# databio/IGD

Measured on AMD Instinct MI355X. Metric: query-intervals/sec (igd search -q, hits-only) on roadmap-scale synthetic .igd, higher is better.
Workload: dtype int32; 1 GPU; BASELINE config 2: roadmap-scale synthetic IGD, 1900 files x 26316 intervals (53143736 tile records, 188505 tiles of 16384 bp, hg38 contigs) replicated per GPU + 1000000 position-sorted queries per step (seed 7), hits-only, queries and DB resident in HBM; queries_per_gpu=1000000, parallelism=query-sharded x1, grouping=sorted, query_layout=contig numbers + starts + ends (12 B/query; igd_hip_search_dev), collective=none

## Files before the change

igd_amd/csrc/engine/host_open.hpp:

```cpp
static thread_local igd_hip_db *t_arenaOwner = nullptr;

template <typename T>
static int dalloc(T **p, size_t n, int64_t *acct)
{
    *p = nullptr;
    if (n == 0) n = 1;
    if (t_arenaOwner && t_arenaOwner->arena) {
        igd_hip_db *o = t_arenaOwner;
        const size_t at = (o->arenaUsed + 255) & ~(size_t)255, bytes = n * sizeof(T);
        if (at + bytes <= o->arenaSize) {
            *p = (T *)(o->arena + at);
            o->arenaUsed = at + bytes;
            if (acct) *acct += (int64_t)bytes;
            return IGD_HIP_OK;
        }
    }
    hipError_t e = hipMalloc((void **)p, n * sizeof(T));
    if (e != hipSuccess) {
        set_err("hipMalloc", e, __FILE__, __LINE__);
        return IGD_HIP_ERR_NOMEM;
    }
    if (acct) *acct += (int64_t)(n * sizeof(T));
    return IGD_HIP_OK;
}
// ... 54 lines not shown
    *got = want;
    return p;
}
extern "C" void igd_hip_free(void *p)
{
    if (!p) return;
    size_t *hdr = (size_t *)((char *)p - 64);
    void *drop = nullptr;
    {
        std::lock_guard<std::mutex> lk(g_pinLock);
        if (g_pinCache && g_pinCacheBytes >= hdr[0]) drop = hdr;
        else { drop = g_pinCache; g_pinCache = hdr; g_pinCacheBytes = hdr[0]; }
    }
    if (drop) (void)hipHostFree(drop);
}
extern "C" const char *igd_hip_scan_kernel_name(void) { return "igd_scan_sorted"; }

extern "C" const char *igd_hip_last_scan_kernel(igd_hip_db *db)
{
    if (db && db->inner) return igd_hip_last_scan_kernel(db->inner);
    if (!db || db->epoch == 0) return "";
    if (db->lastMode == 2) return "igd_scan_tiles";
    if (db->lastDirect) return "igd_scan_direct";
    int32_t uns = 0;
    if (hipSetDevice(db->device) != hipSuccess || hipDeviceSynchronize() != hipSuccess ||
        hipMemcpy(&uns, db->d_ctl + CTL_UNSORTED, 4, hipMemcpyDeviceToHost) != hipSuccess) return "";
    if (uns == db->epoch) return "igd_scan_tiles";
    return db->lastPacked ? "igd_scan_sorted" : "igd_scan_tiles";
}

static double wall_s(void)
{
    struct timespec t;
    clock_gettime(CLOCK_MONOTONIC, &t);
    return (double)t.tv_sec + 1e-9 * (double)t.tv_nsec;
}
#define OPEN_PHASE(name) do { if (tim) { double t_ = wall_s(); fprintf(stderr, "[igd timing]   open: %-22s %8.1f ms\n", name, 1e3 * (t_ - t0)); t0 = t_; } } while (0)

static int build_retiled(igd_hip_db *db, const igd_hip_desc *d, int realShift, const std::vector<Unit> &units, int device)
{
    const int64_t n = db->nRec;
    std::vector<int32_t> st((size_t)n), en((size_t)n), ix((size_t)n), va;
    HIPCHK(hipMemcpy(st.data(), db->d_start, (size_t)n * 4, hipMemcpyDeviceToHost));
    HIPCHK(hipMemcpy(en.data(), db->d_end, (size_t)n * 4, hipMemcpyDeviceToHost));
    HIPCHK(hipMemcpy(ix.data(), db->d_idx, (size_t)n * 4, hipMemcpyDeviceToHost));
    if (db->gType == 1) { va.resize((size_t)n); HIPCHK(hipMemcpy(va.data(), db->d_value, (size_t)n * 4, hipMemcpyDeviceToHost)); }
// ... 71 lines not shown
            snprintf(g_err, sizeof g_err, "igd_hip_open: this libigd_hip.so is a measurement build (IGD_EXP=0x%x) that gives WRONG counts; "
                     "set IGD_HIP_ALLOW_EXP_BUILD=1 to use it anyway", igd_hip_build_flags());
            return IGD_HIP_ERR_ARG;
        }
        fprintf(stderr, "igd_hip: WARNING: measurement build IGD_EXP=0x%x -- counts are WRONG on purpose\n", igd_hip_build_flags());
    }
    std::thread warm;
    try {
        warm = std::thread([device]() {
            int n = 0;
            if (hipGetDeviceCount(&n) == hipSuccess && device >= 0 && device < n && hipSetDevice(device) == hipSuccess) (void)hipFree(nullptr);
        });
    } catch (...) { }
    struct JoinWarm { std::thread &t; ~JoinWarm() { if (t.joinable()) t.join(); } } joinWarm{warm};
    igd_hip_db *db = new igd_hip_db();
    db->device = device;
    {
        const char *fr = getenv("IGD_HIP_RANK");
        db->forceRank = fr && *fr ? atoi(fr) : -1;
        const char *fb = getenv("IGD_HIP_BIG");
        db->bigImage = fb && *fb == '1';
        const char *fd = getenv("IGD_HIP_DIRECT");
        db->forceDirect = fd && *fd ? atoi(fd) : -1;
        db->splitNoStage = getenv("IGD_HIP_SPLIT_NOSTAGE") != nullptr;
        db->splitNoBits = getenv("IGD_HIP_SPLIT_NOBITS") != nullptr;
        db->splitNoRegion = getenv("IGD_HIP_SPLIT_NOREGION") != nullptr;
        db->timing = tim;
    }
    db->nbp = d->nbp; db->gType = d->gType; db->nCtg = d->nCtg; db->nFiles = d->nFiles;
    db->nRec = d->nRecords;

    int64_t nT = 0;
    for (int c = 0; c < d->nCtg; c++) nT += d->nTile[c];
    bool jfits = true;
    for (int c = 0; c < d->nCtg; c++) jfits = jfits && d->nTile[c] < (1 << 27);
    if (nT >= (1 << 27) || !jfits) {
        snprintf(g_err, sizeof g_err, "igd_hip_open: too many tiles (%lld; the engine's limit is 2^27-1)", (long long)nT);
        delete db;
        return IGD_HIP_ERR_ARG;
    }
    db->nT = (int32_t)nT;
    std::vector<int64_t> tileOff((size_t)nT + 1);
    std::vector<int32_t> tileCnt((size_t)nT + 1), tileBd((size_t)nT + 1), ctgBase((size_t)d->nCtg + 1),
        ctgNTile((size_t)d->nCtg + 1), tileUnit0((size_t)nT + 1);
    std::vector<Unit> units;
    int64_t off = 0;
// ... 360 lines not shown
```

igd_amd/csrc/engine/host_search.hpp:

```cpp

static int ensure_workspace(igd_hip_db *db, int64_t nq, int pairBytes)
{
    int rc;
    if (nq > db->wsQueries) {
        HIPCHK(hipDeviceSynchronize());
        if (db->d_fix) (void)hipFree(db->d_fix);
        if (db->d_qw) (void)hipFree(db->d_qw);
        if (db->d_later) (void)hipFree(db->d_later);
        if (db->d_laterHdr) (void)hipFree(db->d_laterHdr);
        db->d_fix = nullptr; db->d_qw = nullptr; db->d_later = nullptr; db->d_laterHdr = nullptr;
        db->wsQueries = 0;
        if ((rc = dalloc(&db->d_fix, (size_t)nq * 2, nullptr)) != IGD_HIP_OK) return rc;
        if ((rc = dalloc(&db->d_qw, (size_t)nq + 64, nullptr)) != IGD_HIP_OK) return rc;
        if ((rc = dalloc(&db->d_later, (size_t)nq + 4096 + 64, nullptr)) != IGD_HIP_OK) return rc;
        if ((rc = dalloc(&db->d_laterHdr, 2 * ((size_t)nq / 256 + 2), nullptr)) != IGD_HIP_OK) return rc;
        db->wsQueries = nq;
    }
    if (pairBytes == 0 || (nq <= db->wsBucket && pairBytes <= db->pairBytes)) return IGD_HIP_OK;
    HIPCHK(hipDeviceSynchronize());
    const int64_t cap = nq > db->wsBucket ? nq : db->wsBucket;
    const int pb = pairBytes > db->pairBytes ? pairBytes : db->pairBytes;
    {
        void *ws[] = { db->d_pairs, db->d_long, db->d_spTable, db->d_spT, db->d_spSub };
        for (void *q : ws) if (q) (void)hipFree(q);
// ... 204 lines not shown
    const int mode = (flags & IGD_HIP_FLAG_SORTED) ? 1 : (flags & IGD_HIP_FLAG_BUCKET) ? 2 : 0;
    const int krule = rule | ((db->v.vshift >= 0 && db->vnest) ? 0x100 : 0);
    const bool packed = db->packed && !(flags & IGD_HIP_FLAG_EXACT) && (!useV || db->packedV);
    if (db->epoch >= 0x3fffffff || db->covStale) {
        HIPCHK(hipMemsetAsync(db->d_spill, 0, ((size_t)db->nT + 2) * 4, st));
        HIPCHK(hipMemsetAsync(db->d_cov, 0, 4 * IGD_COV_LEN(db->nT) * 4, st));
        HIPCHK(hipMemsetAsync(db->d_ctl + CTL_COV, 0, 4 * 4, st));
        if (db->d_spSub && db->spShift >= 0)
            HIPCHK(hipMemsetAsync(db->d_spSub + (((size_t)db->spCoarse * SPF_S) << db->spShift) + db->spCoarse, 0, (size_t)db->spCoarse * 4, st));
        if (!db->covStale) db->epoch = 0;
        db->covStale = false;
    }
    db->epoch++;
    struct StaleGuard { igd_hip_db *d; bool done; ~StaleGuard() { if (!done) d->covStale = true; } } guard{db, false};
    int slot = -1;
    if (db->evOn && db->evUsed < db->evMax && (db->evSeen++ % (db->evEvery > 0 ? db->evEvery : 1)) == 0) slot = db->evUsed++;
    const bool pipeEv = slot >= 0 && slot < IGD_PIPE_EVENTS;
    if (pipeEv) HIPCHK(hipEventRecord(db->ev[4 * slot + 0], st));
    u64 *zh = (flags & IGD_HIP_FLAG_ZERO_FIRST) ? (u64 *)d_hits : nullptr;
    u64 *zt = (flags & IGD_HIP_FLAG_ZERO_FIRST) ? (u64 *)d_total : nullptr;
    const bool direct = mode == 1 && packed && db->ldsHits && db->nWin == 1 && db->v.tileD != nullptr && db->v.vshift < 0 && db->v.shift >= 0 && db->nCtg <= QB_CTG &&
                        (db->forceDirect > 0 || (db->forceDirect < 0 && (flags & IGD_HIP_FLAG_SHORT) && nq >= 28ll * db->nT));
    db->lastDirect = direct ? 1 : 0;
    if (mode != 2) {
        bool vec = ((((uintptr_t)d_ichr) | ((uintptr_t)d_qs) | ((uintptr_t)d_qe)) & 15) == 0;
        const bool fast = packed && db->v.shift >= 0 && db->nCtg <= QB_CTG;
        if (nq < 65536) vec = false;
        bool runsK = d_runs != nullptr && vec && fast;
        if (d_runs && !runsK) {
            if (nq > db->runCap) {
                HIPCHK(hipStreamSynchronize(st));
                if (db->d_runIchr) (void)hipFree(db->d_runIchr);
                db->d_runIchr = nullptr; db->runCap = 0;
                if ((rc = dalloc(&db->d_runIchr, (size_t)nq, nullptr)) != IGD_HIP_OK) return rc;
                db->runCap = nq;
            }
            k_expand_runs<<<(int)((nq + 255) / 256), 256, 0, st>>>(d_runs, db->nCtg, db->d_runIchr, (int)nq);
            d_ichr = db->d_runIchr;
            vec = vec && (((uintptr_t)d_ichr) & 15) == 0;
        }
        const int fillBlocks = (int)((db->nT >> 10) < 256 ? (db->nT >> 10) + 1 : 256);
        const bool wide = vec && nq >= ((int64_t)1 << 22);
#define QB_GRID(PER_) ((int)((nq + (PER_) - 1) / (PER_)) > fillBlocks ? (int)((nq + (PER_) - 1) / (PER_)) : fillBlocks)
#define QB_LAUNCH(VEC_, FAST_, WGT_)                                                                                                  \
    if (direct && FAST_ && runsK && VEC_ == 4)                                         \
        k_query_bounds<4, true, WGT_, true, true><<<QB_GRID(WGT_ * 4), WGT_, 0, st>>>(db->v, d_runs, d_qs, d_qe, (int)nq, krule,      \
        1, db->d_firstQ, db->d_lpos, db->d_fix, db->d_ctl, db->epoch, zh, zt, db->d_qw, db->d_later, db->d_spill,                      \
        (int2 *)db->d_laterHdr, 1);                                                                                                  \
    else if (direct && FAST_)                                                                                                        \
        k_query_bounds<VEC_, true, WGT_, false, true><<<QB_GRID(WGT_ * VEC_), WGT_, 0, st>>>(db->v, d_ichr, d_qs, d_qe, (int)nq, krule, \
        1, db->d_firstQ, db->d_lpos, db->d_fix, db->d_ctl, db->epoch, zh, zt, db->d_qw, db->d_later, db->d_spill,                      \
        (int2 *)db->d_laterHdr, 1);                                                                                                  \
    else if (runsK && VEC_ == 4 && FAST_)                                                                                             \
        k_query_bounds<4, true, WGT_, true><<<QB_GRID(WGT_ * 4), WGT_, 0, st>>>(db->v, d_runs, d_qs, d_qe, (int)nq, krule,            \
        packed ? 1 : 0, db->d_firstQ, db->d_lpos, db->d_fix, db->d_ctl, db->epoch, zh, zt, db->d_qw, db->d_later, db->d_spill,         \
        (int2 *)db->d_laterHdr, mode == 1 ? 1 : 0);                                                                                  \
    else                                                                                                                             \
    k_query_bounds<VEC_, FAST_, WGT_><<<QB_GRID(WGT_ * VEC_), WGT_, 0, st>>>(db->v, d_ichr, d_qs, d_qe, (int)nq, krule,               \
        packed ? 1 : 0, db->d_firstQ, db->d_lpos, db->d_fix, db->d_ctl, db->epoch, zh, zt, db->d_qw, db->d_later, db->d_spill,         \
        (int2 *)db->d_laterHdr, mode == 1 ? 1 : 0)
        if (wide && !direct) { if (fast) QB_LAUNCH(4, true, 1024); else QB_LAUNCH(4, false, 1024); }
        else if (vec) { if (fast) QB_LAUNCH(4, true, 256); else QB_LAUNCH(4, false, 256); }
        else { if (fast) QB_LAUNCH(1, true, 256); else QB_LAUNCH(1, false, 256); }
#undef QB_LAUNCH
#undef QB_GRID
        db->lbShift = wide ? 12 : vec ? 10 : 8;
    }
    if (mode != 1) {
        if (db->spShift >= 0)
            rc = launch_split(db, d_ichr, d_qs, d_qe, (int)nq, krule, mode == 2 ? 0 : db->epoch, packed ? 1 : 0, st,
                              mode == 2 ? zh : nullptr, mode == 2 ? zt : nullptr);
        else
            rc = launch_bucket(db, d_ichr, d_qs, d_qe, (int)nq, krule, mode == 2 ? 0 : db->epoch, packed ? 1 : 0, st,
                                      mode == 2 ? zh : nullptr, mode == 2 ? zt : nullptr);
        if (rc != IGD_HIP_OK) return rc;
    }
    const bool extEv = slot >= 0 && mode == 1 && packed && db->ldsHits && db->nWin == 1;
    if (slot >= 0 && !extEv) HIPCHK(hipEventRecord(db->ev[4 * slot + 1], st));
    ScanArgs a;
    a.firstQ = db->d_firstQ; a.pairN = db->d_pairN; a.pairPos = db->d_pairPos; a.pairs = (const int2 *)db->d_pairs;
    a.walkList = nullptr; a.ctl = db->d_ctl; a.q_ichr = d_ichr; a.q_qs = d_qs; a.q_qe = d_qe; a.q_w = db->d_qw;
    a.total = (u64 *)d_total; a.hitsOut = (u64 *)d_hits;
    a.nq = (int)nq; a.v = v; a.rule = rule; a.epoch = db->epoch; a.mode = mode;
    a.packedWalk = packed ? (useV ? 2 : 1) : 0;
    const int valves = direct ? 8 : (mode != 1 && packed && db->spShift >= 0 ? 1 : 0) | (mode != 2 && packed ? 2 : 0) |
                       (db->bigImage || db->nRec + IGD_CHUNK >= (1ll << 30) ? 4 : 0);
    const size_t tailWave = direct ? (size_t)IGD_D_WLDS : (size_t)IGD_WLDS_BYTES;
    size_t tailLds = (valves & (2 | 8)) ? (size_t)(db->ldsHits ? IGD_TAIL_WG / IGD_WAVE : 4) * tailWave : 0;
    int tailHistOff = -1;
    if ((size_t)db->nFiles * 8 <= (size_t)48 * 1024) { tailHistOff = (int)tailLds; tailLds += (size_t)db->nFiles * 8; }
    if (db->ldsHits) {
        a.out = db->d_slab;
        const SortK K = make_sortk(db, a);
        for (int win = 0; win < db->nWin; win++) {
            const bool last = win == db->nWin - 1;
            const int fileLo = win * db->winN, fileN = db->nWin == 1 ? db->nFiles : (db->nFiles - fileLo < db->winN ? db->nFiles - fileLo : db->winN);
            if (extEv) { db->evStart = db->ev[4 * slot + 1]; db->evStop = db->ev[4 * slot + 2]; }
            if (direct) {
                DirK D;
                D.db = db->v;
                D.a.firstQ = db->d_firstQ; D.a.tileD = db->v.tileD; D.a.q_qs = d_qs; D.a.q_qe = d_qe; D.a.ctl = db->d_ctl; D.a.fix = db->d_fix;
                D.a.heavyS = db->d_heavy + IGD_HEAVY_MAX; D.a.farList = db->d_far; D.a.nq = (int)nq; D.a.v = v; D.a.epoch = db->epoch;
                D.a.rule = rule; D.a.promised = 1; D.a.sbCap = db->sbCap; D.a.wldsBytes = IGD_D_WLDS + 2 * db->sbCap;
                D.a.out = db->d_slab; D.a.hitsOut = (u64 *)d_hits; D.a.totalOut = (u64 *)d_total;
                if (useV) launch_sorted(db, igd_scan_direct<true>, db->grid, IGD_WG_DIR, (size_t)db->ldsDirect, st, D);
                else launch_sorted(db, igd_scan_direct<false>, db->grid, IGD_WG_DIR, (size_t)db->ldsDirect, st, D);
            } else
            launch_scan_any<true>(db, a, useV, packed, st, db->nWin > 1 ? win : -1);
            if (extEv && db->evStart) {
                db->evStart = db->evStop = nullptr;
                HIPCHK(hipEventRecord(db->ev[4 * slot + 1], st)); HIPCHK(hipEventRecord(db->ev[4 * slot + 2], st));
            }
            if (slot >= 0 && last && !extEv) HIPCHK(hipEventRecord(db->ev[4 * slot + 2], st));
            ScanArgs w = a;
            w.out = (u64 *)d_hits;
            SortK Kt = K;
            Kt.a.sbCap = 0; Kt.a.wldsBytes = (int)tailWave; Kt.a.tailHistOff = tailHistOff;
            const int gx = (fileN + IGD_TAIL_WG - 1) / IGD_TAIL_WG;
            dim3 rg(gx, (!last || IGD_REDUCE_GROUPS * gx >= IGD_TAIL_WGS) ? IGD_REDUCE_GROUPS : (IGD_TAIL_WGS + gx - 1) / gx);
            const int rows32 = (mode != 2 && packed) ? db->epoch : 0;
            if (useV)
                k_reduce_slabs<true><<<rg, IGD_TAIL_WG, last ? tailLds : 0, st>>>(Kt, db->d_slab, db->grid, fileN, (u64 *)d_hits + fileLo, (u64 *)d_total,
                                                               db->d_ctl, mode == 1 ? db->epoch : 0, w, db->d_fix, db->d_long, db->d_heavy, last ? valves : -1, rows32);
            else
                k_reduce_slabs<false><<<rg, IGD_TAIL_WG, last ? tailLds : 0, st>>>(Kt, db->d_slab, db->grid, fileN, (u64 *)d_hits + fileLo, (u64 *)d_total,
                                                                db->d_ctl, mode == 1 ? db->epoch : 0, w, db->d_fix, db->d_long, db->d_heavy, last ? valves : -1, rows32);
        }
    } else {
        a.out = (u64 *)d_hits;
// ... 135 lines not shown
```

igd_amd/csrc/engine/measure.hpp:

```cpp
__global__ void k_unit_traffic(DbView db, const int32_t *__restrict__ firstQ, const int32_t *__restrict__ pairN,
                               const int32_t *__restrict__ spill, int epoch, int path ,
                               int rankOK, u64 *__restrict__ acc )
{
    const int u = blockIdx.x * blockDim.x + threadIdx.x;
    u64 nu = 0, nr = 0, np = 0, nd = 0;
    if (u < db.nUnits) {
        const Unit un = db.units[u];
        if (un.n > 0) {
            const int lj = UNIT_J(un);
            const int lb = lj < IGD_SHORT_TILES - 1 ? lj : IGD_SHORT_TILES - 1;
            const bool firstUnit = UNIT_FLAGS(un) & 1;
            if (path == 1) {
                if (firstQ[un.tile + 1] > firstQ[un.tile - lb]) { nu = 1; nr = (u64)un.n; }
            } else if (path == 2) {
                const int f0 = firstQ[un.tile], c0 = firstQ[un.tile + 1] - f0;
                const int cl = spill[un.tile] == epoch ? f0 - firstQ[un.tile - lb] : 0;
                if (c0 | cl) { nu = 1; nr = (u64)un.n; }
                if (firstUnit) {
                    if (rankOK && c0 >= IGD_DENSE_MIN) nd = (u64)c0;
                }
            } else if (pairN[un.tile] != 0) {
                nu = 1; nr = (u64)un.n;
                if (firstUnit) np = (u64)(pairN[un.tile] < 0 ? -pairN[un.tile] : pairN[un.tile]);
            }
// ... 9 lines not shown
        if (nd) atomicAdd(&acc[3], nd);
    }
}

__global__ void k_unit_traffic_direct(DbView db, const int32_t *__restrict__ firstQ, int rule, u64 *__restrict__ acc )
{
    const int u = blockIdx.x * blockDim.x + threadIdx.x;
    u64 nu = 0, nr = 0, nd = 0;
    if (u < db.nUnits) {
        const Unit un = db.units[u];
        const int c0 = firstQ[un.tile + 1] - firstQ[un.tile];
        const bool first = UNIT_FLAGS(un) & 1;
        if (c0 > 0 && c0 <= IGD_HEAVY_FIRST && (un.n > 0 || first)) {
            nd = (u64)c0;
            const bool dead = rule == IGD_HIP_RULE_NEST && un.n == 0;
            if (un.n > 0 || !dead) { nu = 1; nr = (u64)un.n + (first && !dead ? (u64)(db.tileD[un.tile].y & 127) : 0); }
        }
    }
    for (int o = 32; o > 0; o >>= 1) { nu += __shfl_down(nu, o); nr += __shfl_down(nr, o); nd += __shfl_down(nd, o); }
    if ((threadIdx.x & 63) == 0) {
        if (nu) atomicAdd(&acc[0], nu);
        if (nr) atomicAdd(&acc[1], nr);
        if (nd) atomicAdd(&acc[3], nd);
    }
}

extern "C" int igd_hip_batch_traffic(igd_hip_db *db, const int32_t *d_ichr, const int32_t *d_qs, const int32_t *d_qe,
                                     int64_t nq, int32_t v, int rule, int flags, igd_hip_traffic *out)
{
    if (!db || !out || nq < 0 || nq > IGD_MAX_BATCH) return IGD_HIP_ERR_ARG;
    if (db->inner) {
        db->inner->vnest = rule == IGD_HIP_RULE_NEST ? 1 : 0;
        return igd_hip_batch_traffic(db->inner, d_ichr, d_qs, d_qe, nq, v, IGD_HIP_RULE_FLAT, flags, out);
    }
    memset(out, 0, sizeof *out);
    if (nq == 0 || db->nT == 0 || db->nFiles == 0) return IGD_HIP_OK;
    HIPCHK(hipSetDevice(db->device));
    u64 *d_acc = nullptr;
    int64_t *d_h = nullptr;
    int rc;
    if (db->promised && (rc = igd_hip_sync(db, db->stream)) != IGD_HIP_OK) return rc;
    if ((rc = dalloc(&d_acc, 4, nullptr)) != IGD_HIP_OK) return rc;
    if ((rc = dalloc(&d_h, (size_t)db->nFiles + 1, nullptr)) != IGD_HIP_OK) { (void)hipFree(d_acc); return rc; }
    hipStream_t st = db->stream;
    (void)hipMemsetAsync(d_acc, 0, 32, st);
    (void)hipMemsetAsync(d_h, 0, ((size_t)db->nFiles + 1) * 8, st);
    const bool saved = db->evOn;
    db->evOn = false;
    rc = igd_hip_search_dev(db, d_ichr, d_qs, d_qe, nq, v, rule, flags & ~IGD_HIP_FLAG_ZERO_FIRST, d_h, nullptr, st);
    db->evOn = saved;
    int32_t ctl[4] = {0, 0, 0, 0};
    hipError_t e = hipStreamSynchronize(st);
    if (e == hipSuccess) e = hipMemcpy(ctl, db->d_ctl, sizeof ctl, hipMemcpyDeviceToHost);
    if (rc == IGD_HIP_OK && e == hipSuccess) {
        const int mode = (flags & IGD_HIP_FLAG_SORTED) ? 1 : (flags & IGD_HIP_FLAG_BUCKET) ? 2 : 0;
        const bool sortedPath = mode == 1 || (mode == 0 && ctl[CTL_UNSORTED] != db->epoch);
        const bool useV = (v != IGD_HIP_NO_VALUE_FILTER && db->gType == 1);
        const bool packed = db->packed && !(flags & IGD_HIP_FLAG_EXACT) && (!useV || db->packedV);
        const int path = !sortedPath ? 0 : packed ? 2 : 1;
        const bool direct = db->lastDirect != 0 && sortedPath;
        if (direct) k_unit_traffic_direct<<<(db->nUnits + 255) / 256, 256, 0, st>>>(db->v, db->d_firstQ, rule, d_acc);
        else
        k_unit_traffic<<<(db->nUnits + 255) / 256, 256, 0, st>>>(db->v, db->d_firstQ, db->d_pairN, db->d_spill, db->epoch, path,
                                                               ctl[CTL_NOTSTART] != db->epoch ? 1 : 0, d_acc);
        u64 acc[4] = {0, 0, 0, 0};
        e = hipStreamSynchronize(st);
        if (e == hipSuccess) e = hipMemcpy(acc, d_acc, 32, hipMemcpyDeviceToHost);
        const int recB = packed ? (useV ? 8 : 6) : (useV ? 16 : 12);
        out->units = (int64_t)acc[0];
        out->records = (int64_t)acc[1];
        out->record_bytes = (int64_t)acc[1] * recB;
        out->unit_bytes = (int64_t)sizeof(Unit) * db->nUnits + (path == 2 ? 8ll * (db->nT + 1) : sortedPath ? 4ll * (db->nT + 1) : 8ll * db->nT);
        if (direct) out->unit_bytes = (int64_t)(sizeof(Unit) + 8 + 16) * db->nUnits;
        int64_t nLaterWords = 0;
        if (path == 2 && !direct) {
            const int64_t nb = (nq + ((int64_t)1 << db->lbShift) - 1) >> db->lbShift;
            std::vector<int32_t> hdr((size_t)nb * 2);
            e = hipMemcpy(hdr.data(), db->d_laterHdr, (size_t)nb * 8, hipMemcpyDeviceToHost);
            for (int64_t b = 0; b < nb; b++) nLaterWords += hdr[(size_t)b * 2];
        }
        out->query_bytes = direct ? 8ll * (int64_t)acc[3] : path == 2 ? 4ll * nq + 4ll * nLaterWords + 4ll * (int64_t)acc[3]
                         : path == 1 ? 12ll * nq : 8ll * (int64_t)acc[2];
        out->slab_bytes = db->ldsHits ? (int64_t)db->grid * db->nFiles * (path == 2 ? 4 : 8) : 8ll * db->nFiles;
        out->total = out->record_bytes + out->unit_bytes + out->query_bytes + out->slab_bytes;
    }
    (void)hipFree(d_acc); (void)hipFree(d_h);
    (void)igd_hip_sync(db, st);
    if (rc != IGD_HIP_OK) return rc;
    if (e != hipSuccess) { set_err("batch_traffic", e, __FILE__, __LINE__); return IGD_HIP_ERR_DEVICE; }
    return IGD_HIP_OK;
}

__global__ __launch_bounds__(256) void k_copy16(const float4 *__restrict__ in, float4 *__restrict__ outp, size_t n)
{
    size_t i = (size_t)blockIdx.x * blockDim.x + threadIdx.x;
    const size_t stride = (size_t)gridDim.x * blockDim.x;
    for (; i + 3 * stride < n; i += 4 * stride) {
        const float4 a = in[i], b = in[i + stride], c = in[i + 2 * stride], d = in[i + 3 * stride];
        outp[i] = a; outp[i + stride] = b; outp[i + 2 * stride] = c; outp[i + 3 * stride] = d;
    }
    for (; i < n; i += stride) outp[i] = in[i];
}
__global__ __launch_bounds__(256) void k_read16(const float4 *__restrict__ in, size_t n, float *__restrict__ sink)
{
// ... 128 lines not shown
```

igd_amd/csrc/engine/tail.hpp:

```cpp
struct TailHist {
    igd_lds_u64 *p;
    bool on;
    __device__ __forceinline__ void add(int ix, u64 v) const { (void)__hip_atomic_fetch_add(p + ix, v, __ATOMIC_RELAXED, __HIP_MEMORY_SCOPE_WORKGROUP); }
};

template <bool USE_V>
__device__ __forceinline__ void exact_walk_body(const DbView &db, const ScanArgs &a, const int2 *__restrict__ fixList,
                                                const int2 *__restrict__ longList, int gwave, int nwaves, int ctlv, const TailHist hist)
{
    const bool uns = __builtin_amdgcn_readlane(ctlv, CTL_UNSORTED) == a.epoch;
    if (a.mode == 1 && uns) return;
    const bool sortedPath = a.mode == 1 || (a.mode == 0 && !uns);
    const int2 *list = sortedPath ? fixList : longList;
    const int nList = __builtin_amdgcn_readlane(ctlv, (sortedPath ? CTL_NFIX : CTL_NLONG) + (a.epoch & 1));
    const int lane = threadIdx.x & 63;
    u64 found = 0;
    int per = (nList + nwaves - 1) / nwaves;
    per = per > IGD_WAVE ? IGD_WAVE : per;
    for (int l0 = gwave * per; l0 < nList; l0 += nwaves * per) {
        const int cnt = nList - l0 < per ? nList - l0 : per;
        int vq = 0, vkind = -1, vqs = 0, vqe = 0, vn1 = 0, vj1 = -1, vbase = 0, vcnt = 0, voffLo = 0, voffHi = 0, vlob = 0;
        int vu0 = 0, vnu = 0, vqe2 = 0;
        UnitRegs vur;
        vur.offLo = vur.offHi = vur.tile = vur.n = vur.jf = 0;
// ... 329 lines not shown
        if (!(wa.mode == 1 && uns) && (nList > 0 || cov)) {
            hist.on = true;
            for (int f = threadIdx.x; f < K.db.nFiles; f += blockDim.x) hist.p[f] = 0;
            __syncthreads();
        }
    }
    if (!(IGD_EXP & 0x100000)) exact_walk_body<USE_V>(K.db, wa, fixList, longList, gwave, nwaves, ctlv, hist);
    if (!(IGD_EXP & 0x200000)) coverage_body<USE_V>(K.db, wa, d_hits, d_total, gwave, nwaves, ctlv, hist);
    if (hist.on) {
        __syncthreads();
        for (int f = threadIdx.x; f < K.db.nFiles; f += blockDim.x) {
            const u64 c = hist.p[f];
            if (c) atomicAdd(&d_hits[f], c);
        }
    }
    if (valves & 1) heavy_bucket_body<USE_V>(K.db, wa, heavyB, d_hits, d_total, gwave, nwaves, lane, ctlv);
    if (valves & 8) {
        DirArgs d;
        d.firstQ = K.a.firstQ; d.tileD = K.db.tileD; d.q_qs = wa.q_qs; d.q_qe = wa.q_qe; d.ctl = K.a.ctlw; d.fix = nullptr;
        d.heavyS = K.a.heavyS; d.farList = K.a.farList; d.nq = wa.nq; d.v = wa.v; d.epoch = wa.epoch; d.rule = wa.rule;
        d.promised = 1; d.sbCap = 0; d.wldsBytes = K.a.wldsBytes; d.out = nullptr; d.hitsOut = d_hits; d.totalOut = d_total;
        direct_tail_body<USE_V>(K.db, d, smem + (size_t)(threadIdx.x >> 6) * (size_t)K.a.wldsBytes, gwave, nwaves, lane, ctlv);
    } else
    if (valves & 2) {
        unsigned char *wsm = smem + (size_t)(threadIdx.x >> 6) * (size_t)K.a.wldsBytes;
        if (valves & 4) heavy_sorted_body<USE_V, true>(K, d_hits, d_total, wsm, gwave, nwaves, lane, ctlv);
        else {
            const int par = wa.epoch & 1;
            const bool work = (__builtin_amdgcn_readlane(ctlv, CTL_NHEAVYS + par) | __builtin_amdgcn_readlane(ctlv, CTL_NFAR + par)) != 0 &&
                              __builtin_amdgcn_readlane(ctlv, CTL_UNSORTED) != wa.epoch;
            igd_lds_u64 *lh = (K.a.tailHistOff >= 0 && work) ? hist.p : nullptr;
            if (lh) {
                __syncthreads();
                for (int f = threadIdx.x; f < K.db.nFiles; f += blockDim.x) lh[f] = 0;
                __syncthreads();
            }
            if (!(IGD_EXP & 0x10000)) heavy_sorted_body<USE_V, false>(K, d_hits, d_total, wsm, gwave, nwaves, lane, ctlv, lh);
            if (!(IGD_EXP & 0x20000)) far_units_body<USE_V, false>(K, d_hits, d_total, wsm, gwave, nwaves, lane, ctlv, lh);
            if (lh) {
                __syncthreads();
                for (int f = threadIdx.x; f < K.db.nFiles; f += blockDim.x) {
                    const u64 c = lh[f];
                    if (c) atomicAdd(&d_hits[f], c);
                }
            }
        }
// ... 76 lines not shown
```

igd_amd/csrc/igd_hip.hip:

```cpp
#include <hip/hip_runtime.h>
#include <hip/hip_ext.h>
#include <stdint.h>
#include <stdio.h>
#include <stdlib.h>
#include <string.h>
#include <limits.h>
#include <vector>
#include <algorithm>
#include <thread>
#include <mutex>
#include <time.h>
#include <unistd.h>

#include "igd_hip.h"
#include "igd_sortscan.hpp"

#define IGD_WAVE 64
#ifndef IGD_SLOTS
#define IGD_SLOTS 5
#endif
#define IGD_CHUNK (IGD_WAVE * IGD_SLOTS)
#define IGD_SHORT_TILES 4
#ifndef IGD_WPE
#define IGD_WPE 8
// ... 126 lines not shown
    int32_t *d_lpos;
    int32_t *d_cov;
    bool covStale;
    igd_hip_db *inner;
    uint32_t *d_rEmpty;
    int vnest;
    int32_t *d_runIchr;
    int64_t runCap;
    int32_t *d_qw;
    int32_t *d_later;
    int32_t *d_spill;
    int ldsSorted;
    int32_t maxTileCnt;
    int sbCap;
    int32_t *d_laterHdr;
    int lbShift;
    int lastMode, lastPacked;
    int forceRank;
    int forceDirect;
    int4 *d_tileD;
    uint32_t *d_tileBits;
    int ldsDirect;
    int lastDirect;
    bool bigImage;
    bool timing;
    bool splitNoStage, splitNoBits, splitNoRegion;
    uint32_t *d_spTable;
    SpTuple *d_spT;
    uint32_t *d_spSub;
    int spShift, spCoarse;
    char *arena;
    size_t arenaSize, arenaUsed;
    int32_t epoch;
    int32_t promised;
    int32_t *d_pairCnt, *d_pairPos, *d_blockSums;
    void *d_pairs;
    int2 *d_long, *d_fix;
    int32_t *d_ctl;
    int64_t wsQueries;
    int64_t wsBucket;
    int pairBytes;
    u64 *d_slab;
    int grid, ldsBytes;
    bool ldsHits;
    int winN, nWin;
    int64_t *d_qcount, *d_qoff, *d_enumBsum;
// ... 25 lines not shown
    unsigned *d_rsBits;
    int64_t rsUniCap, rsTabCap, rsSizeCap, rsBitsCap;
    u64 *d_coCols, *d_coMat, *d_coA, *d_coB;
    int64_t coColsCap, coMatCap, coACap, coBCap;
    int32_t *d_pmReg;
    long long *d_pmStat;
    int64_t pmRegCap, pmStatCap;
    hipStream_t stream;
    std::vector<hipEvent_t> ev;
    int evMax, evUsed;
    hipEvent_t evStart, evStop;
    int evEvery, evSeen;
    bool evOn;
};


#include "engine/upload.hpp"
#include "engine/query_bounds.hpp"
#include "engine/split.hpp"
#include "engine/compact_image.hpp"
#include "engine/scan_tiles.hpp"
#include "engine/scan_sorted.hpp"
#include "engine/scan_direct.hpp"
#include "engine/tail.hpp"
#include "engine/enumerate_dev.hpp"
#include "engine/hitmap_dev.hpp"
#include "engine/batch_stats_dev.hpp"
#include "engine/sets_dev.hpp"
#include "engine/support_dev.hpp"
#include "engine/coverage_dev.hpp"
#include "engine/member_dev.hpp"
#include "engine/fisher_dev.hpp"
#include "engine/rank_dev.hpp"
#include "engine/restrict_dev.hpp"
#include "engine/cooccur_dev.hpp"
#include "engine/permute_dev.hpp"
#include "engine/host_open.hpp"
#include "engine/host_search.hpp"
#include "engine/host_group.hpp"
#include "engine/host_enumerate.hpp"
#include "engine/seqpare.hpp"
#include "engine/host_misc.hpp"
#include "engine/host_sets.hpp"
#include "engine/host_support.hpp"
#include "engine/host_coverage.hpp"
#include "engine/host_member.hpp"
// ... 11 lines not shown
```

Baseline: 12.78 billion query-intervals/s.

## Add lean short-query scan kernel for sparse sorted query batches

Adds igd_scan_lean_short, a scan path for short, sparse, position-sorted queries. Each wave walks tile units and reads its query range straight from firstQ, instead of going through the later/spill pairing workspace. Heavy tiles and far-previous ranges are pushed to lists that a tail pass handles in slices. Query bounds run in the same bounds-only mode as the direct kernel, and the path is gated by query density thresholds plus an env override. The new path adds code complexity and atomics for the heavy and far lists, and it may only trigger for some batch sizes.

```diff
diff --git a/igd_amd/csrc/engine/host_open.hpp b/igd_amd/csrc/engine/host_open.hpp
--- a/igd_amd/csrc/engine/host_open.hpp
+++ b/igd_amd/csrc/engine/host_open.hpp
@@ -100,6 +100,7 @@
     if (!db || db->epoch == 0) return "";
     if (db->lastMode == 2) return "igd_scan_tiles";
     if (db->lastDirect) return "igd_scan_direct";
+    if (db->lastLeanShort) return "igd_scan_lean_short";
     int32_t uns = 0;
     if (hipSetDevice(db->device) != hipSuccess || hipDeviceSynchronize() != hipSuccess ||
         hipMemcpy(&uns, db->d_ctl + CTL_UNSORTED, 4, hipMemcpyDeviceToHost) != hipSuccess) return "";
@@ -217,6 +218,8 @@
         db->bigImage = fb && *fb == '1';
         const char *fd = getenv("IGD_HIP_DIRECT");
         db->forceDirect = fd && *fd ? atoi(fd) : -1;
+        const char *fl = getenv("IGD_HIP_LEAN_SHORT");
+        db->forceLeanShort = fl && *fl ? atoi(fl) : -1;
         db->splitNoStage = getenv("IGD_HIP_SPLIT_NOSTAGE") != nullptr;
         db->splitNoBits = getenv("IGD_HIP_SPLIT_NOBITS") != nullptr;
         db->splitNoRegion = getenv("IGD_HIP_SPLIT_NOREGION") != nullptr;
diff --git a/igd_amd/csrc/engine/host_search.hpp b/igd_amd/csrc/engine/host_search.hpp
--- a/igd_amd/csrc/engine/host_search.hpp
+++ b/igd_amd/csrc/engine/host_search.hpp
@@ -250,6 +250,16 @@
     const bool direct = mode == 1 && packed && db->ldsHits && db->nWin == 1 && db->v.tileD != nullptr && db->v.vshift < 0 && db->v.shift >= 0 && db->nCtg <= QB_CTG &&
                         (db->forceDirect > 0 || (db->forceDirect < 0 && (flags & IGD_HIP_FLAG_SHORT) && nq >= 28ll * db->nT));
     db->lastDirect = direct ? 1 : 0;
+    bool leanShort = false;
+    if (!direct && mode == 1 && (flags & IGD_HIP_FLAG_SHORT) && packed && db->ldsHits && db->nWin == 1 && db->v.tileD != nullptr && db->v.vshift < 0 &&
+        db->v.shift >= 0 && db->nCtg <= QB_CTG && db->nFiles > 8 && db->forceLeanShort != 0 && db->forceRank <= 0) {
+        const int64_t wavesLean = (int64_t)db->grid * (IGD_WG_LEAN / IGD_WAVE);
+        const bool fits = ((int64_t)db->nUnits + wavesLean - 1) / wavesLean * (IGD_WG_LEAN / IGD_WAVE) * (2 * IGD_LEAN_FIRST) * IGD_CHUNK < (1ll << 32);
+        const bool sparse = db->forceRank == 0 || (nq < 28ll * db->nT && nq >= (int64_t)db->nT);
+        leanShort = fits && (db->forceLeanShort > 0 || (sparse && nq >= (int64_t)(useV ? IGD_LEAN_SHORT_MIN_NQ_V : IGD_LEAN_SHORT_MIN_NQ)));
+    }
+    db->lastLeanShort = leanShort ? 1 : 0;
+    const bool bonly = direct || leanShort;
     if (mode != 2) {
         bool vec = ((((uintptr_t)d_ichr) | ((uintptr_t)d_qs) | ((uintptr_t)d_qe)) & 15) == 0;
         const bool fast = packed && db->v.shift >= 0 && db->nCtg <= QB_CTG;
@@ -271,11 +281,11 @@
         const bool wide = vec && nq >= ((int64_t)1 << 22);
 #define QB_GRID(PER_) ((int)((nq + (PER_) - 1) / (PER_)) > fillBlocks ? (int)((nq + (PER_) - 1) / (PER_)) : fillBlocks)
 #define QB_LAUNCH(VEC_, FAST_, WGT_)                                                                                                  \
-    if (direct && FAST_ && runsK && VEC_ == 4)                                         \
+    if (bonly && FAST_ && runsK && VEC_ == 4)                                         \
         k_query_bounds<4, true, WGT_, true, true><<<QB_GRID(WGT_ * 4), WGT_, 0, st>>>(db->v, d_runs, d_qs, d_qe, (int)nq, krule,      \
         1, db->d_firstQ, db->d_lpos, db->d_fix, db->d_ctl, db->epoch, zh, zt, db->d_qw, db->d_later, db->d_spill,                      \
         (int2 *)db->d_laterHdr, 1);                                                                                                  \
-    else if (direct && FAST_)                                                                                                        \
+    else if (bonly && FAST_)                                                                                                         \
         k_query_bounds<VEC_, true, WGT_, false, true><<<QB_GRID(WGT_ * VEC_), WGT_, 0, st>>>(db->v, d_ichr, d_qs, d_qe, (int)nq, krule, \
         1, db->d_firstQ, db->d_lpos, db->d_fix, db->d_ctl, db->epoch, zh, zt, db->d_qw, db->d_later, db->d_spill,                      \
         (int2 *)db->d_laterHdr, 1);                                                                                                  \
@@ -287,7 +297,7 @@
     k_query_bounds<VEC_, FAST_, WGT_><<<QB_GRID(WGT_ * VEC_), WGT_, 0, st>>>(db->v, d_ichr, d_qs, d_qe, (int)nq, krule,               \
         packed ? 1 : 0, db->d_firstQ, db->d_lpos, db->d_fix, db->d_ctl, db->epoch, zh, zt, db->d_qw, db->d_later, db->d_spill,         \
         (int2 *)db->d_laterHdr, mode == 1 ? 1 : 0)
-        if (wide && !direct) { if (fast) QB_LAUNCH(4, true, 1024); else QB_LAUNCH(4, false, 1024); }
+        if (wide && !bonly) { if (fast) QB_LAUNCH(4, true, 1024); else QB_LAUNCH(4, false, 1024); }
         else if (vec) { if (fast) QB_LAUNCH(4, true, 256); else QB_LAUNCH(4, false, 256); }
         else { if (fast) QB_LAUNCH(1, true, 256); else QB_LAUNCH(1, false, 256); }
 #undef QB_LAUNCH
@@ -311,7 +321,7 @@
     a.total = (u64 *)d_total; a.hitsOut = (u64 *)d_hits;
     a.nq = (int)nq; a.v = v; a.rule = rule; a.epoch = db->epoch; a.mode = mode;
     a.packedWalk = packed ? (useV ? 2 : 1) : 0;
-    const int valves = direct ? 8 : (mode != 1 && packed && db->spShift >= 0 ? 1 : 0) | (mode != 2 && packed ? 2 : 0) |
+    const int valves = direct ? 8 : leanShort ? 16 : (mode != 1 && packed && db->spShift >= 0 ? 1 : 0) | (mode != 2 && packed ? 2 : 0) |
                        (db->bigImage || db->nRec + IGD_CHUNK >= (1ll << 30) ? 4 : 0);
     const size_t tailWave = direct ? (size_t)IGD_D_WLDS : (size_t)IGD_WLDS_BYTES;
     size_t tailLds = (valves & (2 | 8)) ? (size_t)(db->ldsHits ? IGD_TAIL_WG / IGD_WAVE : 4) * tailWave : 0;
@@ -333,6 +343,16 @@
                 D.a.out = db->d_slab; D.a.hitsOut = (u64 *)d_hits; D.a.totalOut = (u64 *)d_total;
                 if (useV) launch_sorted(db, igd_scan_direct<true>, db->grid, IGD_WG_DIR, (size_t)db->ldsDirect, st, D);
                 else launch_sorted(db, igd_scan_direct<false>, db->grid, IGD_WG_DIR, (size_t)db->ldsDirect, st, D);
+            } else
+            if (leanShort) {
+                LsK S;
+                S.db = db->v;
+                S.a.firstQ = db->d_firstQ; S.a.q_qs = d_qs; S.a.q_qe = d_qe; S.a.ctl = db->d_ctl; S.a.fix = db->d_fix;
+                S.a.heavyS = db->d_heavy + IGD_HEAVY_MAX; S.a.farList = db->d_far; S.a.nq = (int)nq; S.a.v = v; S.a.epoch = db->epoch;
+                S.a.rule = rule; S.a.out = db->d_slab; S.a.hitsOut = (u64 *)d_hits; S.a.totalOut = (u64 *)d_total;
+                const size_t l = ((size_t)db->nFiles * 4 + 15) & ~(size_t)15;
+                if (useV) launch_sorted(db, igd_scan_lean_short<true>, db->grid, IGD_WG_LEAN, l, st, S);
+                else launch_sorted(db, igd_scan_lean_short<false>, db->grid, IGD_WG_LEAN, l, st, S);
             } else
             launch_scan_any<true>(db, a, useV, packed, st, db->nWin > 1 ? win : -1);
             if (extEv && db->evStart) {
diff --git a/igd_amd/csrc/engine/measure.hpp b/igd_amd/csrc/engine/measure.hpp
--- a/igd_amd/csrc/engine/measure.hpp
+++ b/igd_amd/csrc/engine/measure.hpp
@@ -55,6 +55,24 @@
         if (nu) atomicAdd(&acc[0], nu);
         if (nr) atomicAdd(&acc[1], nr);
         if (nd) atomicAdd(&acc[3], nd);
+    }
+}
+
+__global__ void k_unit_traffic_lean_short(DbView db, const int32_t *__restrict__ firstQ, int rule, u64 *__restrict__ acc )
+{
+    const int u = blockIdx.x * blockDim.x + threadIdx.x;
+    u64 nu = 0, nr = 0;
+    if (u < db.nUnits) {
+        const Unit un = db.units[u];
+        if (un.n > 0) {
+            const bool hasPrev = UNIT_J(un) > 0 && !(rule == IGD_HIP_RULE_NEST && (UNIT_FLAGS(un) & 2));
+            if (firstQ[un.tile + 1] > firstQ[un.tile - (hasPrev ? 1 : 0)]) { nu = 1; nr = (u64)un.n; }
+        }
+    }
+    for (int o = 32; o > 0; o >>= 1) { nu += __shfl_down(nu, o); nr += __shfl_down(nr, o); }
+    if ((threadIdx.x & 63) == 0) {
+        if (nu) atomicAdd(&acc[0], nu);
+        if (nr) atomicAdd(&acc[1], nr);
     }
 }
 
@@ -92,6 +110,9 @@
         const bool packed = db->packed && !(flags & IGD_HIP_FLAG_EXACT) && (!useV || db->packedV);
         const int path = !sortedPath ? 0 : packed ? 2 : 1;
         const bool direct = db->lastDirect != 0 && sortedPath;
+        const bool leanShort = db->lastLeanShort != 0 && sortedPath;
+        if (leanShort) k_unit_traffic_lean_short<<<(db->nUnits + 255) / 256, 256, 0, st>>>(db->v, db->d_firstQ, rule, d_acc);
+        else
         if (direct) k_unit_traffic_direct<<<(db->nUnits + 255) / 256, 256, 0, st>>>(db->v, db->d_firstQ, rule, d_acc);
         else
         k_unit_traffic<<<(db->nUnits + 255) / 256, 256, 0, st>>>(db->v, db->d_firstQ, db->d_pairN, db->d_spill, db->epoch, path,
@@ -106,13 +127,14 @@
         out->unit_bytes = (int64_t)sizeof(Unit) * db->nUnits + (path == 2 ? 8ll * (db->nT + 1) : sortedPath ? 4ll * (db->nT + 1) : 8ll * db->nT);
         if (direct) out->unit_bytes = (int64_t)(sizeof(Unit) + 8 + 16) * db->nUnits;
         int64_t nLaterWords = 0;
-        if (path == 2 && !direct) {
+        if (leanShort) out->unit_bytes = (int64_t)(sizeof(Unit) + 12) * db->nUnits;
+        if (path == 2 && !direct && !leanShort) {
             const int64_t nb = (nq + ((int64_t)1 << db->lbShift) - 1) >> db->lbShift;
             std::vector<int32_t> hdr((size_t)nb * 2);
             e = hipMemcpy(hdr.data(), db->d_laterHdr, (size_t)nb * 8, hipMemcpyDeviceToHost);
             for (int64_t b = 0; b < nb; b++) nLaterWords += hdr[(size_t)b * 2];
         }
-        out->query_bytes = direct ? 8ll * (int64_t)acc[3] : path == 2 ? 4ll * nq + 4ll * nLaterWords + 4ll * (int64_t)acc[3]
+        out->query_bytes = leanShort ? 8ll * nq : direct ? 8ll * (int64_t)acc[3] : path == 2 ? 4ll * nq + 4ll * nLaterWords + 4ll * (int64_t)acc[3]
                          : path == 1 ? 12ll * nq : 8ll * (int64_t)acc[2];
         out->slab_bytes = db->ldsHits ? (int64_t)db->grid * db->nFiles * (path == 2 ? 4 : 8) : 8ll * db->nFiles;
         out->total = out->record_bytes + out->unit_bytes + out->query_bytes + out->slab_bytes;
diff --git a/igd_amd/csrc/engine/scan_lean_short.hpp b/igd_amd/csrc/engine/scan_lean_short.hpp
--- /dev/null
+++ b/igd_amd/csrc/engine/scan_lean_short.hpp
@@ -0,0 +1,327 @@
+#ifndef IGD_LEAN_SHORT_MIN_NQ
+#define IGD_LEAN_SHORT_MIN_NQ 2000000
+#define IGD_LEAN_SHORT_MIN_NQ_V 1000000
+#endif
+#define WALK_WHOLE 5
+
+struct LsArgs {
+    const int32_t *firstQ;
+    const int32_t *q_qs, *q_qe;
+    int32_t *ctl;
+    int2 *fix;
+    int32_t *heavyS, *farList;
+    int nq, v, epoch, rule;
+    u64 *out;
+    u64 *hitsOut, *totalOut;
+};
+struct LsK { DbView db; LsArgs a; };
+#define KARGL(field) karg_load<decltype(((LsK *)0)->field)>((unsigned)offsetof(LsK, field))
+
+struct LsRegs { int32_t offLo, n, jf, w[IGD_SLOTS], qa, f0, qb; };
+struct LsRaw {
+    uint32_t a[IGD_SLOTS];
+    int32_t x[IGD_SLOTS];
+    int32_t qs, qe;
+    int32_t n;
+};
+
+template <bool USE_V, bool PLAIN>
+__device__ __forceinline__ void ls_issue(const DbView &db, const LsArgs &a, const LsRegs &L, int kk, bool valid, int lane, LsRaw &R)
+{
+    const int kq = PLAIN ? kk : kk & 63;
+    int qa = __builtin_amdgcn_readlane(L.qa, kq), qb = __builtin_amdgcn_readlane(L.qb, kq);
+    int n = __builtin_amdgcn_readlane(L.n, kq);
+    if (!PLAIN && !valid) { qa = 0; qb = 0; n = 0; }
+    R.n = n;
+    const unsigned offLo = (unsigned)__builtin_amdgcn_readlane(L.offLo, kq);
+    const int vo4 = lane * 4, vo2 = lane * 2;
+    const int end = (int)offLo + n;
+    const __amdgpu_buffer_rsrc_t rsA = __builtin_amdgcn_make_buffer_rsrc((void *)db.pse, 0, (int)((unsigned)end * 4u), 0x00020000);
+    if (USE_V) {
+        const __amdgpu_buffer_rsrc_t rsX = __builtin_amdgcn_make_buffer_rsrc((void *)db.pxv, 0, n ? (int)((unsigned)(end + IGD_CHUNK) * 4u) : 0, 0x00020000);
+#pragma unroll
+        for (int r = 0; r < IGD_SLOTS; r++) {
+            R.a[r] = (uint32_t)__builtin_amdgcn_raw_buffer_load_b32(rsA, vo4 + r * 256, (int)(offLo * 4u), 0);
+            R.x[r] = (int)__builtin_amdgcn_raw_buffer_load_b32(rsX, vo4 + r * 256, (int)(offLo * 4u), 0);
+        }
+    } else {
+        const __amdgpu_buffer_rsrc_t rsX = __builtin_amdgcn_make_buffer_rsrc((void *)db.px, 0, n ? (int)((unsigned)(end + IGD_CHUNK) * 2u) : 0, 0x00020000);
+#pragma unroll
+        for (int r = 0; r < IGD_SLOTS; r++) {
+            R.a[r] = (uint32_t)__builtin_amdgcn_raw_buffer_load_b32(rsA, vo4 + r * 256, (int)(offLo * 4u), 0);
+            R.x[r] = (int)(unsigned short)__builtin_amdgcn_raw_buffer_load_b16(rsX, vo2 + r * 128, (int)(offLo * 2u), 0);
+        }
+    }
+    const __amdgpu_buffer_rsrc_t rsS = __builtin_amdgcn_make_buffer_rsrc((void *)a.q_qs, 0, qb * 4, 0x00020000);
+    const __amdgpu_buffer_rsrc_t rsE = __builtin_amdgcn_make_buffer_rsrc((void *)a.q_qe, 0, qb * 4, 0x00020000);
+    R.qs = (int)__builtin_amdgcn_raw_buffer_load_b32(rsS, vo4, qa * 4, 0);
+    R.qe = (int)__builtin_amdgcn_raw_buffer_load_b32(rsE, vo4, qa * 4, 0);
+}
+
+template <bool USE_V, bool GLOBAL, bool KA, int NS>
+__device__ __forceinline__ void ls_compute_n(const DbView &db, const LsArgs &a, const LsRegs &L, int kk, int lane, LsRaw &R, unsigned int *hits32, long long unitNo)
+{
+    const int qa = __builtin_amdgcn_readlane(L.qa, kk), qb = __builtin_amdgcn_readlane(L.qb, kk);
+    const int f0h = __builtin_amdgcn_readlane(L.f0, kk), jf = __builtin_amdgcn_readlane(L.jf, kk);
+    const bool heavy = f0h < 0;
+    const int nl = (f0h & 0x7FFFFFFF) - qa, nE = qb - qa;
+    if (nE <= 0) return;
+    const int W = db.nbp;
+    const int j = jf >> 4;
+    const int T0 = (int)((unsigned)j * (unsigned)W);
+    const bool lister = !GLOBAL && (jf & 1);
+    int cnt[NS];
+#pragma unroll
+    for (int r = 0; r < NS; r++) cnt[r] = 0;
+    if (USE_V) {
+#pragma unroll
+        for (int r = 0; r < NS; r++) {
+            if ((R.x[r] >> 16) < a.v) R.a[r] = 0u;
+            R.x[r] &= 0xFFFF;
+        }
+    }
+    uint32_t Wd[NS];
+#pragma unroll
+    for (int r = 0; r < NS; r++) Wd[r] = (uint32_t)__builtin_amdgcn_readlane(L.w[r], kk);
+    int nLater = 0;
+    auto word = [&](const int p, const int qs_, const int qe_) -> int {
+        const int idx = p + lane;
+        const bool later = idx < nl;
+        const int a0 = qs_ - T0, d_ = qe_ - T0;
+        const int a_ = later ? a0 + W : a0;
+        const bool ok = idx < nE && (unsigned)a_ < (unsigned)W && (unsigned)(d_ - 1) < (unsigned)(later ? W : 2 * W);
+        if (p < nl) nLater += __popcll(__ballot(ok && later));
+        if (lister && p + IGD_WAVE > nl) {
+            const bool inTile = (unsigned)a0 < (unsigned)W || (j == 0 && a0 < 0 && a0 > -W);
+            const bool lst = !later && idx < nE && !ok && inTile;
+            const unsigned long long m = __ballot(lst);
+            if (m) {
+                int32_t *ctl = KA ? KARGL(a.ctl) : a.ctl;
+                int2 *fix = KA ? KARGL(a.fix) : a.fix;
+                const int4 *tileD = KA ? KARGL(db.tileD) : db.tileD;
+                const Unit *units = KA ? KARGL(db.units) : db.units;
+                const int epoch = KA ? KARGL(a.epoch) : a.epoch;
+                const int ctg = tileD[units[unitNo].tile].z;
+                int at = 0;
+                if (lane == 0) at = atomicAdd(&ctl[CTL_NFIX + (epoch & 1)], __popcll(m));
+                at = __builtin_amdgcn_readfirstlane(at);
+                if (lst) fix[at + __popcll(m & ((1ull << lane) - 1ull))] = make_int2(qa + idx, WALK_WHOLE | (ctg << 4));
+            }
+        }
+        const int qe1 = (d_ < W ? d_ : W) + 1;
+        const int w = (int)((unsigned)(65536 - qe1) | ((unsigned)(later ? 1 : a_ + 1) << 16));
+        return (ok && (later || !heavy)) ? w : (int)IGD_NEVER;
+    };
+    auto match = [&](int P0) {
+#pragma unroll
+        for (int r = 0; r < NS; r++) match_slot_asm<false>(cnt[r], Wd[r], P0, R.a[r], 0ull);
+    };
+    const bool cmp = R.n != 0;
+    if (nE > IGD_WAVE) {
+        const int vo4 = lane * 4;
+        const __amdgpu_buffer_rsrc_t rsS = __builtin_amdgcn_make_buffer_rsrc((void *)a.q_qs, 0, qb * 4, 0x00020000);
+        const __amdgpu_buffer_rsrc_t rsE = __builtin_amdgcn_make_buffer_rsrc((void *)a.q_qe, 0, qb * 4, 0x00020000);
+        int w = word(0, R.qs, R.qe);
+        if (cmp) match(w);
+        for (int p = IGD_WAVE; p < nE; p += IGD_WAVE) {
+            const int qs_ = (int)__builtin_amdgcn_raw_buffer_load_b32(rsS, vo4, (qa + p) * 4, 0);
+            const int qe_ = (int)__builtin_amdgcn_raw_buffer_load_b32(rsE, vo4, (qa + p) * 4, 0);
+            w = word(p, qs_, qe_);
+            if (cmp) match(w);
+        }
+    } else {
+        const int w = word(0, R.qs, R.qe);
+        if (cmp) match(w);
+    }
+    if (!cmp) return;
+    if (nLater != 0) {
+#pragma unroll
+        for (int r = 0; r < NS; r++) cnt[r] -= (R.a[r] & 0xFFFFu) == 0xFFFFu ? nLater : 0;
+    }
+    if (GLOBAL) {
+        int t = 0;
+#pragma unroll
+        for (int r = 0; r < NS; r++) {
+            const int c = cnt[r];
+            t += c;
+            if (c) atomicAdd((u64 *)((char *)a.hitsOut + ((size_t)(R.x[r] & 0xFFFF) << 3)), (u64)(unsigned)c);
+        }
+        if (a.totalOut) {
+            for (int o = 32; o > 0; o >>= 1) t += __shfl_down(t, o);
+            if (lane == 0 && t) atomicAdd(a.totalOut, (u64)(unsigned)t);
+        }
+    } else {
+#pragma unroll
+        for (int r = 0; r < NS; r++) {
+            if (!USE_V) {
+                unsigned off;
+                asm("v_mad_u32_u16 %0, %1, 4, 0" : "=v"(off) : "v"(R.x[r]));
+                atomicAdd((unsigned int *)((char *)hits32 + off), (unsigned)cnt[r]);
+            } else atomicAdd(hits32 + R.x[r], (unsigned)cnt[r]);
+        }
+    }
+}
+
+template <bool USE_V, bool GLOBAL, bool KA>
+__device__ __forceinline__ void ls_compute(const DbView &db, const LsArgs &a, const LsRegs &L, int kk, int lane, LsRaw &R, unsigned int *hits32, long long unitNo)
+{
+    const int un = R.n;
+    if (un <= IGD_WAVE) ls_compute_n<USE_V, GLOBAL, KA, 1>(db, a, L, kk, lane, R, hits32, unitNo);
+    else if (un <= 3 * IGD_WAVE) ls_compute_n<USE_V, GLOBAL, KA, 3>(db, a, L, kk, lane, R, hits32, unitNo);
+    else ls_compute_n<USE_V, GLOBAL, KA, IGD_SLOTS>(db, a, L, kk, lane, R, hits32, unitNo);
+}
+
+template <bool USE_V>
+__global__ __launch_bounds__(IGD_WG_LEAN) __attribute__((amdgpu_waves_per_eu(IGD_WPE_LEAN, IGD_WPE_LEAN))) void igd_scan_lean_short(LsK K)
+{
+    const DbView &db = K.db;
+    const LsArgs &a = K.a;
+    if (__builtin_amdgcn_readfirstlane(KARGL(a.ctl)[CTL_UNSORTED]) == KARGL(a.epoch)) return;
+    extern __shared__ __attribute__((aligned(16))) unsigned char smem[];
+    const int lane = threadIdx.x & 63;
+    const int wid = __builtin_amdgcn_readfirstlane((int)(threadIdx.x >> 6));
+    unsigned int *hits = (unsigned int *)smem;
+    {
+        const int nFiles = KARGL(db.nFiles);
+        for (int f = threadIdx.x; f < nFiles; f += IGD_WG_LEAN) hits[f] = 0u;
+    }
+    __syncthreads();
+    constexpr int wavesPerWG = IGD_WG_LEAN / IGD_WAVE;
+    const int gwave = (int)blockIdx.x * wavesPerWG + wid;
+    const int nwaves = gridDim.x * wavesPerWG;
+    LsRaw A, B;
+    const int myUnits = (db.nUnits - gwave + nwaves - 1) / nwaves;
+    const int quarter = (myUnits + 3) >> 2;
+    int prioAt = quarter, prioLevel = 3, done = 0;
+    __builtin_amdgcn_s_setprio(3);
+
+    for (int ub = gwave; ub < db.nUnits; ub += nwaves * IGD_ROUND) {
+        LsRegs L;
+        L.offLo = L.n = L.jf = L.qa = L.f0 = L.qb = 0;
+#pragma unroll
+        for (int r = 0; r < IGD_SLOTS; r++) L.w[r] = 0;
+        {
+            const long long mi = (long long)ub + (long long)lane * nwaves;
+            if (lane < IGD_ROUND && mi < db.nUnits) {
+                const Unit *units = KARGL(db.units);
+                const int32_t *firstQ = KARGL(a.firstQ);
+                const UnitRegs u = load_unit_regs(units + mi);
+                L.offLo = u.offLo; L.jf = u.jf; L.n = u.n;
+#pragma unroll
+                for (int r = 0; r < IGD_SLOTS; r++) L.w[r] = u.w[r];
+                const bool first = u.jf & 1, nest = KARGL(a.rule) == IGD_HIP_RULE_NEST;
+                const int par = KARGL(a.epoch) & 1;
+                if (u.n > 0 || (first && !nest)) {
+                    const bool hasPrev = (u.jf >> 4) > 0 && u.n > 0 && !(nest && (u.jf & 2));
+                    const int f0 = firstQ[u.tile], f1 = firstQ[u.tile + 1], fp = firstQ[u.tile - (hasPrev ? 1 : 0)];
+                    int qa = fp, qb = f1, f0h = f0;
+                    if (f1 - f0 > IGD_LEAN_FIRST) {
+                        if (first) { KARGL(a.heavyS)[atomicAdd(&KARGL(a.ctl)[CTL_NHEAVYS + par], 1)] = u.tile; f0h = f0 | (int)0x80000000; }
+                        else qb = f0;
+                    }
+                    if (f0 - fp > IGD_LEAN_FIRST) {
+                        KARGL(a.farList)[atomicAdd(&KARGL(a.ctl)[CTL_NFAR + par], 1)] = (int)mi;
+                        qa = f0;
+                    }
+                    L.qa = qa; L.f0 = f0h; L.qb = qb;
+                    if (qa >= qb) { L.n = 0; L.qa = L.qb = 0; L.f0 = 0; }
+                } else L.n = 0;
+            }
+        }
+        int cntU = (int)(((long long)db.nUnits - ub + nwaves - 1) / nwaves);
+        if (cntU > IGD_ROUND) cntU = IGD_ROUND;
+        const unsigned long long mVis = __ballot(L.qb > L.qa);
+        if (__popcll(mVis) * 4 < cntU * 3) {
+            unsigned long long m = mVis;
+            int ka = -1, kb = -1;
+            if (m) { ka = __builtin_ctzll(m); m &= m - 1; }
+            if (m) { kb = __builtin_ctzll(m); m &= m - 1; }
+            ls_issue<USE_V, false>(db, a, L, ka < 0 ? 0 : ka, ka >= 0, lane, A);
+            while (ka >= 0) {
+                ls_issue<USE_V, false>(db, a, L, kb < 0 ? 0 : kb, kb >= 0, lane, B);
+                ls_compute<USE_V, false, true>(db, a, L, ka, lane, A, hits, (long long)ub + (long long)ka * nwaves);
+                ka = -1;
+                if (m) { ka = __builtin_ctzll(m); m &= m - 1; }
+                ls_issue<USE_V, false>(db, a, L, ka < 0 ? 0 : ka, ka >= 0, lane, A);
+                if (kb >= 0) ls_compute<USE_V, false, true>(db, a, L, kb, lane, B, hits, (long long)ub + (long long)kb * nwaves);
+                kb = -1;
+                if (m) { kb = __builtin_ctzll(m); m &= m - 1; }
+            }
+            continue;
+        }
+        ls_issue<USE_V, true>(db, a, L, 0, true, lane, A);
+        for (int kk = 0; kk < cntU; kk += 2) {
+            ls_issue<USE_V, true>(db, a, L, kk + 1, true, lane, B);
+            ls_compute<USE_V, false, true>(db, a, L, kk, lane, A, hits, (long long)ub + (long long)kk * nwaves);
+            ls_issue<USE_V, true>(db, a, L, kk + 2, true, lane, A);
+            if (kk + 1 < cntU) ls_compute<USE_V, false, true>(db, a, L, kk + 1, lane, B, hits, (long long)ub + (long long)(kk + 1) * nwaves);
+            done += 2;
+            if (done >= prioAt) {
+                prioAt += quarter;
+                prioLevel--;
+                if (prioLevel == 2) __builtin_amdgcn_s_setprio(2);
+                else if (prioLevel == 1) __builtin_amdgcn_s_setprio(1);
+                else __builtin_amdgcn_s_setprio(0);
+            }
+        }
+    }
+    __syncthreads();
+    {
+        const int nFiles = KARGL(db.nFiles);
+        unsigned int *row32 = (unsigned int *)KARGL(a.out) + (size_t)blockIdx.x * nFiles;
+        for (int f = threadIdx.x; f < nFiles; f += IGD_WG_LEAN) row32[f] = hits[f];
+    }
+}
+
+template <bool USE_V>
+__device__ __forceinline__ void lean_short_tail_body(const DbView &db, const LsArgs &a, int gwave, int nwaves, int lane, int ctlv)
+{
+    if (__builtin_amdgcn_readlane(ctlv, CTL_UNSORTED) == a.epoch) return;
+    int nH = __builtin_amdgcn_readlane(ctlv, CTL_NHEAVYS + (a.epoch & 1));
+    int nF = __builtin_amdgcn_readlane(ctlv, CTL_NFAR + (a.epoch & 1));
+    if (nH == 0 && nF == 0) return;
+    if (nH > IGD_HEAVYS_MAX) nH = IGD_HEAVYS_MAX;
+    if (nF > db.nUnits) nF = db.nUnits;
+    auto run = [&](int u, int qa, int qb, bool later) {
+        const UnitRegs ur = load_unit_regs(db.units + u);
+        LsRegs L;
+        L.offLo = ur.offLo; L.n = ur.n; L.jf = ur.jf;
+#pragma unroll
+        for (int r = 0; r < IGD_SLOTS; r++) L.w[r] = ur.w[r];
+        L.qa = qa; L.qb = qb; L.f0 = later ? qb : qa;
+        if (ur.n == 0) return;
+        LsRaw A;
+        ls_issue<USE_V, true>(db, a, L, 0, true, lane, A);
+        ls_compute<USE_V, true, false>(db, a, L, 0, lane, A, nullptr, u);
+    };
+    int lq0 = 0, lqn = 0, lu0 = 0, lnu = 0;
+    deal_items(nH, gwave, nwaves, lane,
+        [&](int h) {
+            lq0 = lqn = lu0 = lnu = 0;
+            if (h < 0) return 0;
+            const int tl = a.heavyS[h];
+            lq0 = a.firstQ[tl]; lqn = a.firstQ[tl + 1] - lq0;
+            lu0 = db.tileUnit0[tl]; lnu = db.tileUnit0[tl + 1] - lu0;
+            return lnu * ((lqn + IGD_HEAVY_SLICE - 1) / IGD_HEAVY_SLICE);
+        },
+        [&](int hh, int it) {
+            const int q0 = __builtin_amdgcn_readlane(lq0, hh), qn = __builtin_amdgcn_readlane(lqn, hh);
+            const int u0 = __builtin_amdgcn_readlane(lu0, hh), nu = __builtin_amdgcn_readlane(lnu, hh);
+            const int sc = it / nu, fs = q0 + sc * IGD_HEAVY_SLICE;
+            run(u0 + it % nu, fs, fs + (qn - sc * IGD_HEAVY_SLICE < IGD_HEAVY_SLICE ? qn - sc * IGD_HEAVY_SLICE : IGD_HEAVY_SLICE), false);
+        });
+    deal_items(nF, gwave, nwaves, lane,
+        [&](int h) {
+            lq0 = lqn = lu0 = 0;
+            if (h < 0) return 0;
+            lu0 = a.farList[h];
+            const int tl = db.units[lu0].tile;
+            lq0 = a.firstQ[tl - 1]; lqn = a.firstQ[tl] - lq0;
+            return (lqn + IGD_HEAVY_SLICE - 1) / IGD_HEAVY_SLICE;
+        },
+        [&](int hh, int it) {
+            const int q0 = __builtin_amdgcn_readlane(lq0, hh), qn = __builtin_amdgcn_readlane(lqn, hh);
+            const int fs = q0 + it * IGD_HEAVY_SLICE;
+            run(__builtin_amdgcn_readlane(lu0, hh), fs, fs + (qn - it * IGD_HEAVY_SLICE < IGD_HEAVY_SLICE ? qn - it * IGD_HEAVY_SLICE : IGD_HEAVY_SLICE), true);
+        });
+}
diff --git a/igd_amd/csrc/engine/tail.hpp b/igd_amd/csrc/engine/tail.hpp
--- a/igd_amd/csrc/engine/tail.hpp
+++ b/igd_amd/csrc/engine/tail.hpp
@@ -375,6 +375,13 @@
         d.promised = 1; d.sbCap = 0; d.wldsBytes = K.a.wldsBytes; d.out = nullptr; d.hitsOut = d_hits; d.totalOut = d_total;
         direct_tail_body<USE_V>(K.db, d, smem + (size_t)(threadIdx.x >> 6) * (size_t)K.a.wldsBytes, gwave, nwaves, lane, ctlv);
     } else
+    if (valves & 16) {
+        LsArgs d;
+        d.firstQ = K.a.firstQ; d.q_qs = wa.q_qs; d.q_qe = wa.q_qe; d.ctl = K.a.ctlw; d.fix = nullptr;
+        d.heavyS = K.a.heavyS; d.farList = K.a.farList; d.nq = wa.nq; d.v = wa.v; d.epoch = wa.epoch; d.rule = wa.rule;
+        d.out = nullptr; d.hitsOut = d_hits; d.totalOut = d_total;
+        lean_short_tail_body<USE_V>(K.db, d, gwave, nwaves, lane, ctlv);
+    } else
     if (valves & 2) {
         unsigned char *wsm = smem + (size_t)(threadIdx.x >> 6) * (size_t)K.a.wldsBytes;
         if (valves & 4) heavy_sorted_body<USE_V, true>(K, d_hits, d_total, wsm, gwave, nwaves, lane, ctlv);
diff --git a/igd_amd/csrc/igd_hip.hip b/igd_amd/csrc/igd_hip.hip
--- a/igd_amd/csrc/igd_hip.hip
+++ b/igd_amd/csrc/igd_hip.hip
@@ -172,6 +172,8 @@
     uint32_t *d_tileBits;
     int ldsDirect;
     int lastDirect;
+    int forceLeanShort;
+    int lastLeanShort;
     bool bigImage;
     bool timing;
     bool splitNoStage, splitNoBits, splitNoRegion;
@@ -243,6 +245,7 @@
 #include "engine/scan_tiles.hpp"
 #include "engine/scan_sorted.hpp"
 #include "engine/scan_direct.hpp"
+#include "engine/scan_lean_short.hpp"
 #include "engine/tail.hpp"
 #include "engine/enumerate_dev.hpp"
 #include "engine/hitmap_dev.hpp"
```

New measurement: 12.55 billion query-intervals/s. -1.8%, worse.
